# qpc001/Feature_Base_Pointcloud_Registration

Hardware: AMD Instinct MI355X
Metric: registered scans/sec + pose RMSE vs ref, 64×1800 synthetic Velodyne (higher is better)
Workload: dtype f32; 1 GPU; C2: 64x1800 HDL-64-style scans, ~100k-pt local corner+surf map; 1024 independent scan-to-map jobs per GPU per step (C4-style independent jobs); parallelism=single GPU, imu_deskew=False, exact_voxel_order=0

## Files before the change

### feature_base_pointcloud_registration_amd/api.py

```python
import ctypes
import os

import numpy as np

from .fbr_types import (DESKEW_TABLE, IMU_SAMPLE, KEYPOSE, PF_FLOAT32, POINT_XYZI, POINT_XYZIRT, REG_STATS, FbrParams,
                        FbrRegStats, PointCloud2, default_params, ptr)

_HERE = os.path.dirname(os.path.abspath(__file__))
_LIB = None
_VP = ctypes.c_void_p
_I64 = ctypes.c_int64
_I32 = ctypes.c_int32

EXPORTED_SYMBOLS = [
    "fbr_params_default", "fbr_strerror", "fbr_abi_version", "fbr_device_count", "fbr_create",
    "fbr_destroy", "fbr_set_map", "fbr_get_map", "fbr_project", "fbr_extract_features",
    "fbr_register", "fbr_register_trace", "fbr_process_scan", "fbr_reset_stream",
    "fbr_process_batch", "fbr_ingest_bytes", "fbr_debug_counters", "fbr_map_grid_info", "fbr_batch_stage", "fbr_batch_launch", "fbr_batch_wait",
    "fbr_batch_flush", "fbr_batch_export_ready", "fbr_batch_results", "fbr_batch_set_full_masks", "fbr_batch_labels", "fbr_batch_export", "fbr_batch_bytes", "fbr_set_profiling", "fbr_set_profiling_kernels", "fbr_kernel_time", "fbr_stream",
    "fbr_voxel_grid", "fbr_affine_from_pose", "fbr_pose_from_affine", "fbr_selftest_math", "fbr_selftest_eigen6", "fbr_selftest_eig_certified", "fbr_selftest_voxel_order", "fbr_selftest_radix_sort",
    "fbr_load_map", "fbr_pcd_read", "fbr_pcd_write_ascii", "fbr_pcd_write_binary",
    "fbr_msg_to_points", "fbr_points_to_msg_data", "fbr_project_msg", "fbr_process_msg",
    "fbr_imu_convert", "fbr_imu_deskew_info", "fbr_set_deskew", "fbr_stream_copy_bandwidth", "fbr_valu_peak",
    "fbr_keyframe_params_default", "fbr_keyframes_add", "fbr_keyframes_set_pose", "fbr_keyframes_count",
# ... 457 lines not shown
        _check(lib().fbr_ingest_bytes(self._h, ctypes.byref(v)), "fbr_ingest_bytes")
        return v.value

    def batch_stage(self, scans, guesses):
        keep, arr, n_in = self._scan_ptrs(scans)
        g = np.ascontiguousarray(np.asarray(guesses, np.float32).reshape(-1, 6))
        _check(lib().fbr_batch_stage(self._h, arr, ptr(n_in), len(keep), ptr(g)), "fbr_batch_stage")
        self._staged = len(keep)

    def batch_launch(self):
        _check(lib().fbr_batch_launch(self._h), "fbr_batch_launch")

    def batch_wait(self):
        _check(lib().fbr_batch_wait(self._h), "fbr_batch_wait")

    def batch_results(self):
        poses = np.zeros((self._staged, 6), np.float32)
        stats = np.zeros(self._staged, REG_STATS)
        _check(lib().fbr_batch_results(self._h, ptr(poses), ptr(stats)), "fbr_batch_results")
        return poses, stats

    def batch_set_full_masks(self, on=True):
        _check(lib().fbr_batch_set_full_masks(self._h, int(bool(on))), "fbr_batch_set_full_masks")

    def batch_labels(self, job):
        n = _I64()
        rc = lib().fbr_batch_labels(self._h, int(job), None, 0, ctypes.byref(n))
        if rc not in (0, -4):
            _check(rc, "fbr_batch_labels")
        out = np.zeros(max(n.value, 1), np.int8)
        _check(lib().fbr_batch_labels(self._h, int(job), ptr(out), len(out), ctypes.byref(n)), "fbr_batch_labels")
        return out[:n.value]

    def batch_export(self, device_ptr):
        _check(lib().fbr_batch_export(self._h, ctypes.c_void_p(device_ptr)), "fbr_batch_export")

    def batch_flush(self):
        _check(lib().fbr_batch_flush(self._h), "fbr_batch_flush")

    def batch_export_ready(self, device_ptr, wait_stream=0):
        st, lid = _VP(), _I64()
        _check(lib().fbr_batch_export_ready(self._h, ctypes.c_void_p(device_ptr), ctypes.c_void_p(wait_stream or None),
                                            ctypes.byref(st), ctypes.byref(lid)), "fbr_batch_export_ready")
        return lid.value, st.value or 0

    def diag_ring_filter(self, kernel):
        f = lib().fbr_diag_ring_filter
        f.restype, f.argtypes = ctypes.c_int, [_VP, ctypes.c_int]
        _check(f(self._h, int(kernel)), "fbr_diag_ring_filter")

    def diag_force_capacity_error(self, job):
        f = lib().fbr_diag_force_capacity_error
        f.restype, f.argtypes = ctypes.c_int, [_VP, ctypes.c_int]
        _check(f(self._h, int(job)), "fbr_diag_force_capacity_error")

    def batch_bytes(self):
        t, g = ctypes.c_double(), ctypes.c_double()
        _check(lib().fbr_batch_bytes(self._h, ctypes.byref(t), ctypes.byref(g)), "fbr_batch_bytes")
        return t.value, g.value

    def set_profiling(self, on=True, kernels=None):
        names = None if not kernels else ",".join(kernels).encode()
        _check(lib().fbr_set_profiling_kernels(self._h, names), "fbr_set_profiling_kernels")
        _check(lib().fbr_set_profiling(self._h, 1 if on else 0), "fbr_set_profiling")

    def kernel_time(self, name):
# ... 47 lines not shown
```

### feature_base_pointcloud_registration_amd/csrc/fbr_api.hip

```cpp
#include <hip/hip_runtime.h>

#include <algorithm>
#include <atomic>
#include <chrono>
#include <condition_variable>
#include <cmath>
#include <cstdio>
#include <cstdlib>
#include <cstring>
#include <dlfcn.h>
#include <functional>
#include <map>
#include <mutex>
#include <set>
#include <string>
#include <thread>
#include <vector>

#include "fbr_common.h"
#include "fbr_imu.h"
#include "fbr_kernels.h"
#include "fbr_msg.h"

using namespace fbr;
// ... 169 lines not shown
  int8_t* d_fits = nullptr;
  int8_t* d_nsame = nullptr;
  int32_t* d_fb_list = nullptr;
  int32_t* d_bin = nullptr;
  int64_t bin_nb = 0, bin_nb_c = 0;
  unsigned long long* h_iter_flags = nullptr;
  unsigned long long* d_iter_flags = nullptr;
  unsigned long long gn_gen = 0;
  std::set<std::string> profile_only;
  int32_t* d_iter_cnt = nullptr;
  unsigned char* d_feat_scratch = nullptr;
  uint8_t* d_msg = nullptr;
  uint64_t msg_cap = 0;
  bool crop_cached = false;
  bool crop_join = false;
  int32_t* h_crop = nullptr;
  float* h_guess = nullptr;
  int max_items = 0;
  float* d_pose_out = nullptr;
  fbr_reg_stats* d_stats = nullptr;
  float* d_trace = nullptr;
  bool has_map = false;
  DevGrid grid_c, grid_s;
  std::vector<fbr_point_xyzi> map_c_host, map_s_host;
  bool have_projection = false;
  int staged_B = 0;
  std::vector<int64_t> staged_nin;
  double time_last = -1.0;
  bool profiling = false;
  std::map<std::string, KernelTimer> timers;
  std::vector<int32_t> last_iters, last_q, last_n, last_m;
  int items_hint = 0;
  unsigned long long* d_feat_stamps = nullptr;
  fbr_deskew_table* d_desk = nullptr;
  int32_t* d_desk_mode = nullptr;
  int32_t* d_rowmin = nullptr;
  int32_t* d_choff = nullptr;
  DevArena arena;
  bool desk_any = false;
  bool no_time_call = false;
  std::vector<fbr_keypose> kf_poses;
  std::vector<int64_t> kf_c_off, kf_c_cnt, kf_s_off, kf_s_cnt;
  float4 *d_kf_c = nullptr, *d_kf_s = nullptr;
  int64_t kf_c_cap = 0, kf_s_cap = 0, kf_c_used = 0, kf_s_used = 0;
  float4 *d_kraw_c = nullptr, *d_kraw_s = nullptr;
  int64_t kraw_c_cap = 0, kraw_s_cap = 0;
  float4 *d_kds_c = nullptr, *d_kds_s = nullptr;
  int64_t kds_c_n = 0, kds_s_n = 0;
  KfSeg* d_kf_segs = nullptr;
  int64_t kf_segs_cap = 0;
  int* d_bounds = nullptr;
  bool map_nocrop = false;
  int stream_degenerate = 0;
  JobResult* d_result = nullptr;
  JobResult* h_result = nullptr;
  fbr_point_xyzirt* h_scan = nullptr;
  int64_t* h_nin = nullptr;
  uint8_t* h_msg = nullptr;
  uint64_t h_msg_cap = 0;
  Ingest ing;
  JobResult* h_direct = nullptr;
  JobResult* d_direct = nullptr;
  int32_t* d_direct_done = nullptr;
  int32_t direct_gen = 0;
  int32_t direct_gen_seq = 0;
  bool tail_pending = false;
// ... 206 lines not shown
    desk = DeskArgs{c->d_desk_mode + i0, c->d_desk + i0, c->d_rowmin + j0 * c->H};
  const float4* pk = (!sb.stream_mode && !desk.mode && c->staged_pk) ? c->staged_pk + i0 * c->NMAX : nullptr;
  if (!sb.stream_mode && !pk && !c->staged_24) return FBR_ERR_STATE;
  int32_t* owner = c->d_owner + j0 * c->HW;
  OwnerTag ot;
  const int trc = next_owner_tag(c, &ot);
  if (trc) return trc;
  TIMED_ON(c, sb.st, "project", launch_project(sb.st, c->d_pts + i0 * c->NMAX, c->d_nin + i0, c->NMAX, sb.B, c->H,
                                               c->W, owner, c->d_err + j0, sb.stream_mode ? c->single_n : -1, pk, ot));
  TIMED_ON(c, sb.st, "extract",
           launch_extract(sb.st, c->d_pts + i0 * c->NMAX, c->NMAX, owner, sb.B, c->H, c->W, c->d_rowcnt + j0 * c->H,
                          c->d_choff + j0 * c->H * (c->W / 32 + 1),
                          c->d_cloud + j0 * c->HW, c->d_col + j0 * c->HW, c->d_range + j0 * c->HW,
                          c->d_start + j0 * c->H, c->d_end + j0 * c->H, c->d_nvalid + j0, desk, pk, ot));
  return FBR_OK;
}

bool packed_scans_enabled() {
  static const bool v = [] {
    const char* e = std::getenv("FBR_PACKED_SCANS");
    return e ? std::atoi(e) != 0 : true;
  }();
  return v;
}

bool feat_surf_window() {
  static const bool v = [] {
    const char* e = std::getenv("FBR_FEAT_SURF_WINDOW");
    return e ? std::atoi(e) != 0 : true;
  }();
  return v;
}

int stage_features(fbr_ctx* c, const Sub& sb, bool stream_mode, bool err_clear = false, bool labels_out = false) {
  const int64_t j0 = sb.j0, HW = c->HW, H = c->H;
  FeatArgs a{};
  a.B = sb.B;
  a.H = c->H;
  a.W = c->W;
  a.cloud = c->d_cloud + j0 * HW;
  a.col = c->d_col + j0 * HW;
  a.range = c->d_range + j0 * HW;
  a.start_ring = c->d_start + j0 * H;
  a.end_ring = c->d_end + j0 * H;
  a.nvalid = c->d_nvalid + j0;
  a.edge_thr = c->P.edge_threshold;
  a.surf_thr = c->P.surf_threshold;
  if (stream_mode) {
    a.stream = c->d_sstream;
    a.label = c->d_label_stream;
  } else {
    CK(hipMemsetAsync(c->d_sstate + j0, 0, sizeof(StreamState) * sb.B, sb.st));
    a.stream = c->d_sstate + j0;
    a.label = c->d_label + j0 * HW;
  }
  a.corner_slot = c->d_corner_slot + j0 * H * kCornerPerRing;
  a.corner_cnt = c->d_corner_cnt + j0 * H;
  a.err = c->d_err + j0;
  a.surf_full = labels_out || !feat_surf_window() ? 1 : 0;
  a.carry = stream_mode ? 1 : 0;
  a.fresh = stream_mode ? 0 : 1;
  feat_caps(c->W, a);
  a.gscratch = c->d_feat_scratch + j0 * H * a.gslot_bytes;
  a.stamps = c->d_feat_stamps ? c->d_feat_stamps + j0 * H * 12 : nullptr;
  if (!err_clear) CK(hipMemsetAsync(c->d_err + j0, 0, sizeof(int32_t) * sb.B, sb.st));
  TIMED_ON(c, sb.st, "features", launch_features(sb.st, a));
  if (!stream_mode && c->diag_err_job >= sb.in0 && c->diag_err_job < sb.in0 + sb.B)
    CK(hipMemsetD32Async((hipDeviceptr_t)(c->d_err + j0 + (c->diag_err_job - sb.in0)), 1, 1, sb.st));
  VgRing v{};
  v.cloud = a.cloud;
  v.label = a.label;
  v.start_ring = a.start_ring;
  v.end_ring = a.end_ring;
  v.B = sb.B;
  v.H = c->H;
  v.HW = HW;
  v.cap = c->W;
  v.leaf = c->P.odometry_surf_leaf_size;
  v.out = c->d_surf_ring + j0 * HW;
  v.stride_out = c->W;
  v.cnt_out = c->d_surf_ring_cnt + j0 * H;
  v.dbg = std::getenv("FBR_VR_DBG") ? std::atoi(std::getenv("FBR_VR_DBG")) : 0;
  v.exact = c->P.exact_voxel_order ? 1 : 0;
  v.stamps = a.stamps;
  v.kernel = c->diag_ring_filter;
  TIMED_ON(c, sb.st, "voxel_ring", launch_voxel_ring(sb.st, v));
  TIMED_ON(c, sb.st, "concat",
           launch_concat(sb.st, sb.B, c->H, c->W, a.corner_slot, a.corner_cnt, v.out, v.cnt_out,
                         c->d_corner_all + j0 * HW, HW, c->d_ncorner + j0, c->d_surf_all + j0 * HW, HW,
                         c->d_nsurf + j0, c->d_ring_box + j0 * H * kRingBox));
  c->ring_box_valid = true;
  return FBR_OK;
}

GnArgs gn_args(fbr_ctx* c, const Sub& sb, bool trace) {
  const int64_t j0 = sb.j0, HW = c->HW, ib = j0 * c->items_per_job;
  const int mi = std::max(1, c->P.max_iterations);
// ... 911 lines not shown
  if (hipMemset(c->d_sstream, 0, sizeof(StreamState)) != hipSuccess ||
      hipMemset(c->d_label_stream, 0, HW) != hipSuccess || hipMemset(c->d_col, 0, sizeof(int32_t) * Bw * HW) != hipSuccess ||
      hipMemset(c->d_range, 0, sizeof(float) * Bw * HW) != hipSuccess ||
      hipMemset(c->d_desk_mode, 0, sizeof(int32_t) * B) != hipSuccess ||
      hipMemset(c->d_owner, 0x7F, sizeof(int32_t) * Bw * HW) != hipSuccess) {
    fbr_destroy(c);
    return FBR_ERR_HIP;
  }
  c->owner_ib = 1;
  while (((int64_t)1 << c->owner_ib) < c->NMAX) ++c->owner_ib;
  c->owner_tmax = (owner_tags_enabled() && c->owner_ib <= 24) ? ((uint32_t)kEmptyOwner >> c->owner_ib) - 1 : 0;
  if (const char* e = std::getenv("FBR_OWNER_TMAX"))
    if (c->owner_tmax && std::atoi(e) > 0) c->owner_tmax = std::min<uint32_t>(c->owner_tmax, (uint32_t)std::atoi(e));
  *out = c;
  return FBR_OK;
}

int fbr_destroy(fbr_ctx* c) {
  if (!c) return FBR_ERR_INVALID_ARG;
  (void)hipSetDevice(c->dev);
  if (c->stream) (void)fbr_sync(c->stream);
  for (int k = 1; k < kMaxSub; ++k)
    if (c->xstream[k]) (void)fbr_sync(c->xstream[k]);
  void* ptrs[] = {c->d_pts, c->d_nin, c->d_guess, c->d_owner, c->d_rowcnt, c->d_col, c->d_start, c->d_end,
                  c->d_nvalid, c->d_cloud, c->d_range, c->d_sstate, c->d_sstream, c->d_label, c->d_label_stream,
                  c->d_corner_slot, c->d_corner_cnt, c->d_surf_ring, c->d_surf_ring_cnt, c->d_ring_box,
                  c->d_err, c->d_corner_all, c->d_surf_all, c->d_cornerDS, c->d_surfDS, c->d_ncorner, c->d_nsurf,
                  c->d_ncds, c->d_nsds, c->d_vg_scratch, c->d_gn, c->d_items, c->d_nitems,
                  c->d_item_range, c->d_cropcnt, c->d_cropwork, c->d_partial, c->d_pose_out, c->d_stats, c->d_trace, c->d_nbr, c->d_fitc, c->d_fits, c->d_nsame, c->d_fb_list, c->d_bin, c->d_iter_cnt, c->d_feat_scratch, c->d_msg,
                  c->d_desk, c->d_desk_mode, c->d_rowmin, c->d_choff,
                  c->d_kf_c, c->d_kf_s, c->d_kraw_c, c->d_kraw_s, c->d_kds_c, c->d_kds_s, c->d_kf_segs, c->d_bounds, c->d_direct_done, c->d_pk};
  for (void* p : ptrs)
    if (p) (void)hipFree(p);
  if (c->h_iter_flags) (void)hipHostFree(c->h_iter_flags);
  free_grid(c->grid_c);
  free_grid(c->grid_s);
  arena_free(c->arena);
  for (void* h : {(void*)c->h_result, (void*)c->h_scan, (void*)c->h_nin, (void*)c->h_msg, (void*)c->h_crop, (void*)c->h_guess,
                  (void*)c->h_direct})
    if (h) (void)hipHostFree(h);
  if (c->d_result) (void)hipFree(c->d_result);
  if (c->ing.cstream) (void)fbr_sync(c->ing.cstream);
  if (c->ing.xstream) (void)fbr_sync(c->ing.xstream);
  if (c->ing.h_stage) (void)hipHostFree(c->ing.h_stage);
  if (c->ing.d_pts_slot[1]) (void)hipFree(c->ing.d_pts_slot[1]);
  for (uint8_t* d : c->ing.d_stage)
    if (d) (void)hipFree(d);
  if (c->ing.copied_ev) (void)hipEventDestroy(c->ing.copied_ev);
  if (c->ing.d_nin) (void)hipFree(c->ing.d_nin);
  if (c->ing.h_nin) (void)hipHostFree(c->ing.h_nin);
  for (auto& e : c->ing.up_ev)
    if (e) (void)hipEventDestroy(e);
  for (auto& e : c->ing.chunk_ev)
    if (e) (void)hipEventDestroy(e);
  if (c->ing.cstream) (void)hipStreamDestroy(c->ing.cstream);
  if (c->ing.xstream) (void)hipStreamDestroy(c->ing.xstream);
  for (auto& kv : c->timers) {
    for (auto& pr : kv.second.pending) {
      (void)hipEventDestroy(pr.first);
      (void)hipEventDestroy(pr.second);
    }
    for (auto& pr : kv.second.pool) {
      (void)hipEventDestroy(pr.first);
      (void)hipEventDestroy(pr.second);
    }
  }
// ... 984 lines not shown
  return FBR_OK;
}

int fbr_ingest_bytes(fbr_ctx* c, double* h2d_bytes) {
  if (!c || !h2d_bytes) return FBR_ERR_INVALID_ARG;
  *h2d_bytes = c->ing.h2d_bytes;
  return FBR_OK;
}

int fbr_voxel_grid(fbr_ctx* c, const fbr_point_xyzi* in, int64_t n, float leaf, fbr_point_xyzi* out, int64_t* n_out) {
  if (!c || n < 0 || (n && !in) || !(leaf > 0)) return FBR_ERR_INVALID_ARG;
  CK(enter(c));
  std::vector<fbr_point_xyzi> o;
  int rc = voxel_grid_once(c, in, n, leaf, o);
  if (rc) return rc;
  if (out) std::memcpy(out, o.data(), sizeof(fbr_point_xyzi) * o.size());
  if (n_out) *n_out = (int64_t)o.size();
  return FBR_OK;
}

extern "C" int fbr_diag_feature_stamps(fbr_ctx* c, unsigned long long* out ) {
  if (!c) return FBR_ERR_INVALID_ARG;
  CK(enter(c));
  const size_t n = (size_t)c->Bwork * c->H * 12;
  if (!c->d_feat_stamps) {
    CK(hipMalloc(&c->d_feat_stamps, sizeof(unsigned long long) * n));
    CK(hipMemset(c->d_feat_stamps, 0, sizeof(unsigned long long) * n));
    return FBR_OK;
  }
  if (out) CK(fbr_memcpy_sync(out, c->d_feat_stamps, sizeof(unsigned long long) * n, hipMemcpyDeviceToHost));
  return FBR_OK;
}

int fbr_set_profiling(fbr_ctx* c, int enable) {
  if (!c) return FBR_ERR_INVALID_ARG;
  c->profiling = enable != 0;
  return FBR_OK;
}

int fbr_set_profiling_kernels(fbr_ctx* c, const char* names) {
  if (!c) return FBR_ERR_INVALID_ARG;
  c->profile_only.clear();
  if (!names) return FBR_OK;
  std::string cur;
  for (const char* q = names;; ++q) {
    if (*q == ',' || *q == '\0') {
      if (!cur.empty()) c->profile_only.insert(cur);
      cur.clear();
      if (*q == '\0') break;
    } else {
      cur.push_back(*q);
    }
  }
  return FBR_OK;
}

int fbr_kernel_time(fbr_ctx* c, const char* kernel, double* total_ms, int64_t* launches) {
  if (!c || !kernel) return FBR_ERR_INVALID_ARG;
  CK(enter(c));
  auto itr = c->timers.find(kernel);
  if (itr == c->timers.end()) {
    if (total_ms) *total_ms = 0.0;
    if (launches) *launches = 0;
    return FBR_OK;
  }
  KernelTimer& t = itr->second;
// ... 213 lines not shown
```

### feature_base_pointcloud_registration_amd/csrc/fbr_kernels.h

```cpp
#pragma once
#include <hip/hip_ext.h>
#include <hip/hip_runtime.h>
#include <stdint.h>

#include <algorithm>
#include <atomic>

#include "fbr_common.h"

namespace fbr {

struct LaunchTimer {
  hipEvent_t start = nullptr, stop = nullptr;
  int launched = 0;
};
inline LaunchTimer& launch_timer() {
  static thread_local LaunchTimer t;
  return t;
}

struct DebugCounters {
  std::atomic<long long> launches{0}, host_syncs{0}, flag_polls{0};
  std::atomic<long long> host_ns[4] = {0, 0, 0, 0};
  std::atomic<long long> batch_ns[2] = {0, 0};
// ... 38 lines not shown
struct DeskArgs {
  const int32_t* mode;
  const fbr_deskew_table* table;
  int32_t* rowmin;
};
void launch_extract(hipStream_t s, const fbr_point_xyzirt* pts, int64_t nmax, int32_t* owner, int B, int H,
                    int W, int32_t* rowcnt, int32_t* choff, float4* cloud, int32_t* col, float* range,
                    int32_t* start_ring, int32_t* end_ring, int32_t* nvalid, const DeskArgs& desk,
                    const float4* pk, const OwnerTag& ot);

struct FeatArgs {
  int B, H, W;
  const float4* cloud;
  const int32_t* col;
  const float* range;
  const int32_t* start_ring;
  const int32_t* end_ring;
  const int32_t* nvalid;
  float edge_thr, surf_thr;
  StreamState* stream;
  int8_t* label;
  float4* corner_slot;
  int32_t* corner_cnt;
  int32_t* err;
  int lcap, segcap;
  int kseg;
  int nwcap;
  unsigned char* gscratch;
  int64_t gslot_bytes;
  unsigned long long* stamps;
  int surf_full = 1;
  int carry = 0;
  int fresh = 0;
};
size_t features_lds_bytes(const FeatArgs& a, int nwv);
size_t features_gslot_bytes(const FeatArgs& a);
void launch_features(hipStream_t s, const FeatArgs& a);

struct VgSet {
  const float4* in;
  int64_t stride_in;
  const int32_t* cnt_in;
  int64_t cap;
  float4* out;
  int64_t stride_out;
  int32_t* cnt_out;
  uint32_t* scratch;
  float leaf;
  int nseg;
  int morton;
  int exact;
  const float* box;
  int box_n;
  int64_t box_stride;
};
constexpr int64_t kVgScratch = 5;
struct VgArgs {
  VgSet s[2];
  int32_t* err = nullptr;
};
constexpr int32_t kVgErrLookback = 16;
constexpr int64_t kVgLdsCap = 4096;
void launch_voxel_grid(hipStream_t s, const VgArgs& a);

struct DevArena {
  char* base = nullptr;
// ... 166 lines not shown
```

### feature_base_pointcloud_registration_amd/csrc/k_features.hip

```cpp
#include "fbr_common.h"
#include "fbr_kernels.h"
#include "fbr_sort.h"

#include <algorithm>
#include <cstdlib>
#include <type_traits>

namespace fbr {

__device__ __forceinline__ void wsync() {
  __builtin_amdgcn_fence(__ATOMIC_SEQ_CST, "workgroup");
  __builtin_amdgcn_wave_barrier();
}

namespace {
constexpr uint64_t kPadKey = kF64KeyMax;
constexpr int kSurfWindow = 64;
constexpr int kWin = 256 + 16;
constexpr int kWinBytes = kWin * (sizeof(float) + sizeof(int16_t));
}

struct Bits {
  uint64_t* w;
  __device__ __forceinline__ bool get(int i) const { return (w[i >> 6] >> (i & 63)) & 1ull; }
// ... 111 lines not shown
                              const FeatArgs& a, int job, const uint64_t* frz = nullptr) {
  const int nwm = (m >> 6) + 1;
  uint32_t cmr[WMAX];
#pragma unroll
  for (int w = 0; w < WMAX; ++w) cmr[w] = (w < nwm && 64 * w + lane <= m) ? cmbits(64 * w + lane) : 0u;
  for (int round = 0;; ++round) {
    bool any = false, progress = false;
#pragma unroll
    for (int w = 0; w < WMAX; ++w) {
      const uint64_t live = frz ? und[w] & ~frz[w] : und[w];
      if (w < nwm && live != 0ull) {
        bool nt = false, tk = false;
        const bool mine = (live >> lane) & 1ull;
        if (mine) {
          const uint32_t wt = win10(w > 0 ? tak[w - 1] : 0ull, tak[w], w + 1 < WMAX ? tak[w + 1] : 0ull, lane);
          const uint32_t wu = win10(w > 0 ? und[w - 1] : 0ull, und[w], w + 1 < WMAX ? und[w + 1] : 0ull, lane);
          if (wt & cmr[w]) nt = true;
          else if (!(wu & cmr[w])) tk = true;
        }
        const uint64_t bt = __ballot(tk);
        tak[w] |= bt;
        if (bt != 0ull && mine && !tk && !nt) {
          const uint32_t wt = win10(w > 0 ? tak[w - 1] : 0ull, tak[w], w + 1 < WMAX ? tak[w + 1] : 0ull, lane);
          nt = (wt & cmr[w]) != 0u;
        }
        const uint64_t bn = __ballot(nt);
        und[w] &= ~(bt | bn);
        progress |= (bt | bn) != 0ull;
        any |= (frz ? und[w] & ~frz[w] : und[w]) != 0ull;
      }
    }
    if (!any || (frz && !progress)) break;
    if (round > 4 * (m + 2)) {
      if (lane == 0) atomicOr(&a.err[job], 8);
      break;
    }
  }
}

__device__ __forceinline__ int wave_partition(SmoothEntry* a, int lo, int hi, float p, uint16_t* posL, uint16_t* posR,
                                              int lane) {
  int cntL = 0;
  for (int b = lo; b < hi; b += 64) {
    const int i = b + lane;
    const bool isL = i < hi && !(a[i].v < p);
    const uint64_t bl = __ballot(isL);
    if (isL) posL[cntL + __popcll(bl & ((1ull << lane) - 1ull))] = (uint16_t)i;
    cntL += __popcll(bl);
  }
  int cntR = 0;
  for (int t = hi - 1; t >= lo; t -= 64) {
    const int i = t - lane;
    const bool isR = i >= lo && !(p < a[i].v);
    const uint64_t br = __ballot(isR);
    if (isR) posR[cntR + __popcll(br & ((1ull << lane) - 1ull))] = (uint16_t)i;
    cntR += __popcll(br);
  }
  wsync();
  const int mn = min(cntL, cntR);
  int K1 = 0;
  for (int k0 = 0; k0 < mn; k0 += 64) {
    const int k = k0 + lane;
    const uint64_t bo = __ballot(k < mn && posL[k] < posR[k]);
    K1 += __popcll(bo);
    if (bo != ~0ull) break;
  }
// ... 352 lines not shown
    uint64_t mk = S.occc.w[c] | A;
#pragma unroll
    for (int d = 1; d <= 5; ++d) mk |= (A >> d) | (An << (64 - d));
#pragma unroll
    for (int d = 1; d <= 6; ++d) mk |= (B << d) | (Bp >> (64 - d));
    if (c == 0 && S.wlo == 0)
      for (int k = 0; k < 5 && k < S.L; ++k)
        if (st->picked04[k]) mk |= 1ull << k;
    S.picked.w[c] = mk;
  }
  __syncthreads();
  FBR_STAMP(1);

  int corner_cnt = 0;
  float4* corner_out = a.corner_slot + (int64_t)slot * kCornerPerRing;
  constexpr int kCq = WMAX;
  float cpf[kCq];
  int pf_seg = -1, pf_next = -1, pf_len = 0;
  auto prefetch_curv = [&](int j0) __attribute__((always_inline)) {
    pf_next = -1;
    for (int jj = j0; jj < 6; ++jj) {
      const int psp = (s * (6 - jj) + e * jj) / 6, pep = (s * (5 - jj) + e * (jj + 1)) / 6 - 1;
      if (psp >= pep) continue;
      const int pb = max(psp - S.wlo - 6, 0), pl = min(pep - S.wlo + 7, S.L) - pb;
      if (pl > 64 * kCq || pep - psp + 1 > segcap) return;
#pragma unroll
      for (int q = 0; q < kCq; ++q) cpf[q] = S.gcurv[pb + min(64 * q + lane, pl - 1)];
      pf_next = jj;
      pf_len = pl;
      return;
    }
  };
  int lastj = -1;
  for (int j = 0; j < 6; j++)
    if ((s * (6 - j) + e * j) / 6 < (s * (5 - j) + e * (j + 1)) / 6 - 1) lastj = j;
  for (int j = 0; j < 6; j++) {
    const int sp = (s * (6 - j) + e * j) / 6;
    const int ep = (s * (5 - j) + e * (j + 1)) / 6 - 1;
    if (sp >= ep) continue;
    const int m = ep - sp;
    if (m + 1 > segcap || m > kseg) {
      if (tid == 0) atomicOr(&a.err[job], 2);
      return;
    }
    S.sbase = max(sp - S.wlo - 6, 0);
    const int slen = min(ep - S.wlo + 7, S.L) - S.sbase;
    if (pf_seg != j)
      for (int t = tid; t < slen; t += NT) S.scurv[t] = S.gcurv[S.sbase + t];
    __syncthreads();
#ifdef FBR_FEAT_SKIP_STALE
    const bool has_stale = false;
#else
    const bool has_stale = (sp <= 4 && 4 < ep);
#endif
    auto sorted_order = [&]() __attribute__((always_inline)) {
      int kpow = 1;
      while (kpow < m) kpow <<= 1;
      for (int t = lane; t < kpow; t += 64) {
        uint64_t key = kPadKey;
        if (t < m) {
          const int pos = sp + t;
          const float v = (pos == 4) ? st->smooth4_value : S.scurv[pos - S.wlo - S.sbase];
          key = ((uint64_t)__float_as_uint(v) << 16) | (uint64_t)t;
        }
        S.keys[t] = key;
      }
      wsync();
      bitonic_sort_keys<QP>(S.keys, kpow, lane);
      bool tflag = false, nflag = false;
      for (int t = lane; t < m; t += 64) {
        const uint32_t vb = (uint32_t)(S.keys[t] >> 16);
        nflag |= vb > 0x7f800000u;
        if (t + 1 < m) tflag |= (uint32_t)(S.keys[t + 1] >> 16) == vb;
      }
      const bool nan = __any(nflag);
      const bool tie = __any(tflag) || nan;
      FBR_STAMP(2);
      if (tie) {
        SmoothEntry* A = nan ? S.seg : (SmoothEntry*)S.rb;
        for (int t = lane; t < m; t += 64) {
          const int pos = sp + t;
          A[t] = (pos == 4) ? SmoothEntry{st->smooth4_value, st->smooth4_ind} : SmoothEntry{S.scurv[pos - S.wlo - S.sbase], pos};
        }
        wsync();
        if (nan) {
          if (lane == 0) std_sort_emul(S.seg, m, S.sstack);
          wsync();
        } else {
// ... 49 lines not shown
        }
        wsync();
      }
    };
    float* tlv = (float*)S.rb;
    uint16_t* tlu = (uint16_t*)(tlv + segcap);
    uint16_t* vis = tlu + segcap;
    auto cm_member = [&](int u) __attribute__((always_inline)) -> bool {
      const int li = sp - S.wlo + u;
      const int f = reach_fwd(S, li), b = reach_bwd(S, li);
      float cv[11];
#pragma unroll
      for (int d = 0; d < 11; ++d) cv[d] = S.scurv[max(li + d - 5, 0) - S.sbase];
      const float vu = cv[5];
      const int lf = min(f, m - u), lb = min(b, u);
      const uint32_t nbf = ((1u << lf) - 1u) << 5, nbb = ((1u << lb) - 1u) << (5 - lb);
      const uint32_t epb = (m - u >= 1 && m - u <= 5) ? 1u << (4 + m - u) : 0u;
      uint32_t gt = 0, eq = 0;
#pragma unroll
      for (int d = 1; d <= 5; ++d) {
        gt |= (cv[5 + d] > vu ? 1u : 0u) << (4 + d);
        eq |= (!(cv[5 + d] < vu || cv[5 + d] > vu) ? 1u : 0u) << (4 + d);
        gt |= (cv[5 - d] > vu ? 1u : 0u) << (5 - d);
        eq |= (!(cv[5 - d] < vu || cv[5 - d] > vu) ? 1u : 0u) << (5 - d);
      }
      const uint32_t notep = u != m ? ~0u : 0u;
      const uint32_t nb = nbf | nbb;
      const uint32_t hc = ((gt | epb) & nbf) | (gt & nbb & notep);
      S.cm[u] = hc | (nb << 10) | ((uint32_t)f << 20) | ((uint32_t)b << 24);
      return ((eq & ~epb & nbf) | (eq & nbb & notep)) != 0u;
    };
    const bool seg_full = a.surf_full || (a.carry && sp <= 9);
    const bool cm_sparse = !seg_full && !has_stale;
    bool direct = !has_stale;
#ifdef FBR_FEAT_SKIP_CM
    if (direct) {
      for (int u = tid; u <= m; u += NT) S.cm[u] = 0u;
      __syncthreads();
    }
    if (false) {
#else
    if (direct) {
#endif
      bool tf = false;
      int nlist = m + 1;
      if (cm_sparse) {
        uint16_t* list = (uint16_t*)S.rb;
        if (wv == 0) {
          int cnt = 0;
          const int wlo_u = j == lastj ? m + 1 : max(0, m - (kSurfWindow - 1));
          for (int k0 = 0; k0 <= m; k0 += 64) {
            const int u = k0 + lane;
            bool need = false;
            if (u <= m) {
              const int li = sp + u - S.wlo;
              need = u >= wlo_u || (!S.picked.get(li) && S.edgec.get(li));
            }
            const uint64_t bm = __ballot(need);
            if (need) list[cnt + __popcll(bm & ((1ull << lane) - 1ull))] = (uint16_t)u;
            cnt += __popcll(bm);
          }
          if (lane == 0) S.tmask[15] = (uint64_t)cnt;
        }
        if constexpr (NWV == 1) wsync();
        else __syncthreads();
        nlist = (int)S.tmask[15];
      }
      for (int k0 = 64 * wv; k0 < nlist; k0 += NT) {
        if (cm_sparse) {
          const int k = k0 + lane;
          if (k < nlist) tf |= cm_member(((const uint16_t*)S.rb)[k]);
        } else {
          const int u = k0 + lane;
          if (u <= m) tf |= cm_member(u);
        }
      }
      if constexpr (NWV == 1) {
        direct = !__any(tf);
        wsync();
      } else {
        __syncthreads();
        direct = !__syncthreads_or(tf);
      }
      FBR_STAMP(10);
    }
    if (wv == 0) {
    if (!direct) sorted_order();
    FBR_STAMP(3);
    if (has_stale) {
      SmoothEntry* ent = (SmoothEntry*)S.rb;
      for (int k = lane; k <= m; k += 64) ent[k] = S.seg[k];
      wsync();
      if (!stale_walks_fast(S, slen, ent, a, m, CL, corner_out, corner_cnt, S.cm,
                               (int32_t*)(ent + segcap), lane)) {
        if (lane == 0) serial_walks(S, slen, ent, a, job, m, CL, corner_out, corner_cnt);
        corner_cnt = __shfl(corner_cnt, 0);
        wsync();
      }
    } else {
      uint64_t und[WMAX], tak[WMAX];
      auto corner_walk = [&]() __attribute__((always_inline)) {
#pragma unroll
        for (int w = 0; w < WMAX; ++w) {
          const int u = 64 * w + lane;
          bool cand = false;
          if (u <= m) {
            const int li = sp + u - S.wlo;
            cand = !S.picked.get(li) && S.edgec.get(li);
          }
          und[w] = __ballot(cand);
          tak[w] = 0ull;
        }
#ifndef FBR_FEAT_SKIP_CORNER
        greedy_rounds(m, lane, und, tak, [&](int u) { return S.cm[u] & 1023u; }, a, job);
#endif
      };
      corner_walk();
      FBR_STAMP(4);
      int T = 0;
      if (direct) {
#pragma unroll
        for (int w = 0; w < WMAX; ++w) {
          if ((tak[w] >> lane) & 1ull) {
            const int q = T + __popcll(tak[w] & ((1ull << lane) - 1ull));
            const int u = 64 * w + lane;
            tlu[q] = (uint16_t)u;
            tlv[q] = S.scurv[sp + u - S.wlo - S.sbase];
          }
          T += __popcll(tak[w]);
        }
        wsync();
        bool tf = false;
        for (int c = lane; c < T; c += 64) {
          const int u = tlu[c];
          const float vu = tlv[c];
          int rank = 0;
          for (int c2 = 0; c2 < T; ++c2) {
            const int u2 = tlu[c2];
            const float v2 = tlv[c2];
            if (u2 == m) rank += (u != m);
            else if (u != m && c2 != c) {
              if (v2 > vu) ++rank;
              else if (!(v2 < vu)) tf = true;
            }
          }
          vis[rank] = (uint16_t)u;
        }
        if (__any(tf)) {
          direct = false;
          wsync();
          sorted_order();
          corner_walk();
        }
        wsync();
        FBR_STAMP(11);
      }
      if (lane < WMAX) {
        uint64_t t = 0;
#pragma unroll
        for (int w = 0; w < WMAX; ++w)
          if (w == lane) t = tak[w];
        S.tmask[lane] = t;
      }
      wsync();
      const int R = direct ? T : m + 1;
      int taken = 0;
      for (int r0 = 0; r0 < R && taken < kCornerPerSeg; r0 += 64) {
        const int rr = r0 + lane;
        int u = -1;
        if (rr < R) u = direct ? (int)vis[rr] : (int)S.sorder[rr == 0 ? m : m - rr];
        const bool acc = u >= 0 && ((S.tmask[u >> 6] >> (u & 63)) & 1ull);
        const uint64_t mk = __ballot(acc);
        const int pos = taken + __popcll(mk & ((1ull << lane) - 1ull));
        if (acc && pos < kCornerPerSeg) {
          corner_out[corner_cnt + pos] = CL[sp + u];
          const int li = sp + u - S.wlo;
          const uint32_t c = S.cm[u];
          atomicOr((unsigned long long*)&S.labpos.w[li >> 6], 1ull << (li & 63));
          or_range(S.picked, li - (int)((c >> 24) & 15u), li + (int)((c >> 20) & 15u));
        }
        taken += __popcll(mk);
      }
      corner_cnt += min(taken, kCornerPerSeg);
      wsync();
      FBR_STAMP(5);
      if constexpr (NWV == 1) prefetch_curv(j + 1);
      const bool bnd = !seg_full;
      const int ulo = bnd ? max(0, m - (kSurfWindow - 1)) : 0;
      auto surf_cand = [&](bool window) __attribute__((always_inline)) {
#pragma unroll
        for (int w = 0; w < WMAX; ++w) {
          const int u = 64 * w + lane;
          bool cand = false;
          if (u <= m && (!window || u >= ulo - 5)) {
            const int li = sp + u - S.wlo;
            cand = !S.picked.get(li) && S.surfc.get(li);
          }
          und[w] = __ballot(cand);
          tak[w] = 0ull;
        }
      };
      auto surf_cm = [&](int u) {
        const uint32_t c = S.cm[u];
        return ((c >> 10) & 1023u) & ~(c & 1023u);
      };
      if (bnd && j == lastj) {
#pragma unroll
        for (int w = 0; w < WMAX; ++w) tak[w] = 0ull;
      } else {
        surf_cand(bnd && ulo > 0);
#ifndef FBR_FEAT_SKIP_SURF
        if (bnd && ulo > 0) {
          uint64_t frz[WMAX];
#pragma unroll
          for (int w = 0; w < WMAX; ++w) {
            const int u = 64 * w + lane;
            frz[w] = und[w] & __ballot(u < ulo);
          }
          greedy_rounds(m, lane, und, tak, surf_cm, a, job, frz);
          bool open = false;
#pragma unroll
          for (int w = 0; w < WMAX; ++w) {
            const int u = 64 * w + lane;
            open |= u >= m - 4 && u <= m && ((und[w] >> lane) & 1ull) && !((frz[w] >> lane) & 1ull);
          }
          if (__any(open)) {
            if (direct) {
              bool tf2 = false;
              for (int u = lane; u <= m; u += 64) tf2 |= cm_member(u);
              wsync();
              if (__any(tf2)) sorted_order();
            }
            surf_cand(false);
            greedy_rounds(m, lane, und, tak, surf_cm, a, job);
          }
        } else {
          greedy_rounds(m, lane, und, tak, surf_cm, a, job);
        }
#endif
      }
      FBR_STAMP(6);
#pragma unroll
      for (int w = 0; w < WMAX; ++w) {
        const int u = 64 * w + lane;
        if (u <= m && ((tak[w] >> lane) & 1ull)) {
          const int li = sp + u - S.wlo;
          const uint32_t c = S.cm[u];
          atomicOr((unsigned long long*)&S.labneg.w[li >> 6], 1ull << (li & 63));
          or_range(S.picked, li - (int)((c >> 24) & 15u), li + (int)((c >> 20) & 15u));
        }
      }
      pf_seg = pf_next;
      if (pf_seg >= 0) {
#pragma unroll
        for (int q = 0; q < kCq; ++q)
          if (64 * q + lane < pf_len) S.scurv[64 * q + lane] = cpf[q];
      }
      wsync();
    }
    FBR_STAMP(7);
    FBR_STAMP(8);
    }
    if constexpr (NWV > 1) __syncthreads();
  }
  if constexpr (NWV > 1) __syncthreads();
  int8_t* LB = a.label + job * HW;
  for (int k = max(cb, 0) + tid; k < ca; k += NT) {
    const int li = k - S.wlo;
    const int8_t lab = S.labpos.get(li) ? 1 : (S.labneg.get(li) ? -1 : 0);
    if (k >= 5 && k < n - 5) LB[k] = lab;
    else if (k < 5 && (lab != 0 || a.fresh)) LB[k] = lab;
  }
  if (cb <= 0 && tid < 5 && tid < S.L) st->picked04[tid] = S.picked.get(tid) ? 1 : 0;
  if (tid == 0) a.corner_cnt[slot] = corner_cnt;
#ifdef FBR_FEAT_STAMPS
  FBR_STAMP(9);
  if (tid == 0 && a.stamps)
    for (int i = 0; i < 12; ++i) a.stamps[(int64_t)slot * 12 + i] = stamp_acc[i];
#endif
}

size_t features_lds_bytes(const FeatArgs& a, int nwv) {
  const size_t region_b = std::max<size_t>((size_t)nwv * kWinBytes, (size_t)8 * a.segcap + sizeof(int32_t) * kCornerPerSeg);
  return (size_t)((a.segcap + 19) & ~3) * sizeof(float) + (size_t)9 * a.nwcap * sizeof(uint64_t) + sizeof(uint64_t) * 16 +
         sizeof(SortFrame) * kSortStack + sizeof(uint32_t) * a.segcap + 16 + region_b;
}

size_t features_gslot_bytes(const FeatArgs& a) {
  const size_t b = sizeof(uint64_t) * a.kseg + 2 * sizeof(SmoothEntry) * a.segcap + 2 * sizeof(uint16_t) * a.segcap +
                   16 + sizeof(float) * a.lcap;
  return (b + 255) & ~(size_t)255;
}

int feature_waves(int rings) {
  static const int forced = [] {
    const char* e = std::getenv("FBR_FEAT_WAVES");
    const int v = e ? std::atoi(e) : 0;
    return v >= 4 ? 4 : v >= 2 ? 2 : v == 1 ? 1 : 0;
  }();
  if (forced) return forced;
  return rings <= 2048 ? 4 : 1;
}

void launch_features(hipStream_t s, const FeatArgs& a) {
  const int nwv = feature_waves(a.B * a.H);
  const dim3 grid(a.B * a.H);
  if (nwv == 1 && a.segcap <= 5 * 64 && a.kseg <= 4 * 128) {
// ... 18 lines not shown
```

Baseline: 142,700 scans/s.

## Add compacted-candidate greedy selection for corner and surface feature picking

Adds a compact path in the feature kernel. Corner candidates are gathered into a dense list of at most 128, and the greedy non-maximum suppression rounds run over one or two 64-bit masks using precomputed 11-bit neighbour conflict masks, instead of sweeping WMAX words over the whole segment. Surface selection in the bounded window gets the same treatment and falls back to the generic path when the window is still open. The surface window default becomes 59 and the path is switched by env vars. Also adds a diagnostic path-record buffer and API, which is off unless allocated.

```diff
diff --git a/feature_base_pointcloud_registration_amd/api.py b/feature_base_pointcloud_registration_amd/api.py
--- a/feature_base_pointcloud_registration_amd/api.py
+++ b/feature_base_pointcloud_registration_amd/api.py
@@ -513,6 +513,15 @@
         _check(lib().fbr_batch_labels(self._h, int(job), ptr(out), len(out), ctypes.byref(n)), "fbr_batch_labels")
         return out[:n.value]
 
+    def feature_paths(self):
+        f = lib().fbr_diag_feature_paths
+        f.restype, f.argtypes = ctypes.c_int, [_VP, _VP, _I64, _VP]
+        n = _I64()
+        _check(f(self._h, None, 0, ctypes.byref(n)), "fbr_diag_feature_paths")
+        out = np.zeros(max(n.value, 1), np.uint32)
+        _check(f(self._h, ptr(out), len(out), ctypes.byref(n)), "fbr_diag_feature_paths")
+        return out[:n.value].reshape(-1, self.params.n_scan)
+
     def batch_export(self, device_ptr):
         _check(lib().fbr_batch_export(self._h, ctypes.c_void_p(device_ptr)), "fbr_batch_export")
 
diff --git a/feature_base_pointcloud_registration_amd/csrc/fbr_api.hip b/feature_base_pointcloud_registration_amd/csrc/fbr_api.hip
--- a/feature_base_pointcloud_registration_amd/csrc/fbr_api.hip
+++ b/feature_base_pointcloud_registration_amd/csrc/fbr_api.hip
@@ -225,6 +225,7 @@
   std::vector<int32_t> last_iters, last_q, last_n, last_m;
   int items_hint = 0;
   unsigned long long* d_feat_stamps = nullptr;
+  uint32_t* d_feat_paths = nullptr;
   fbr_deskew_table* d_desk = nullptr;
   int32_t* d_desk_mode = nullptr;
   int32_t* d_rowmin = nullptr;
@@ -497,6 +498,24 @@
   return v;
 }
 
+bool feat_compact() {
+  static const bool v = [] {
+    const char* e = std::getenv("FBR_FEAT_COMPACT");
+    return e ? std::atoi(e) != 0 : true;
+  }();
+  return v;
+}
+
+constexpr int kFeatSurfWinDefault = 59;
+int feat_surf_win() {
+  static const int v = [] {
+    const char* e = std::getenv("FBR_FEAT_SURF_WIN");
+    const int w = e ? std::atoi(e) : kFeatSurfWinDefault;
+    return w == 59 ? 59 : 64;
+  }();
+  return v;
+}
+
 int stage_features(fbr_ctx* c, const Sub& sb, bool stream_mode, bool err_clear = false, bool labels_out = false) {
   const int64_t j0 = sb.j0, HW = c->HW, H = c->H;
   FeatArgs a{};
@@ -528,6 +547,9 @@
   feat_caps(c->W, a);
   a.gscratch = c->d_feat_scratch + j0 * H * a.gslot_bytes;
   a.stamps = c->d_feat_stamps ? c->d_feat_stamps + j0 * H * 12 : nullptr;
+  a.compact = feat_compact() ? 1 : 0;
+  a.surf_win = feat_surf_win();
+  a.paths = c->d_feat_paths ? c->d_feat_paths + j0 * H : nullptr;
   if (!err_clear) CK(hipMemsetAsync(c->d_err + j0, 0, sizeof(int32_t) * sb.B, sb.st));
   TIMED_ON(c, sb.st, "features", launch_features(sb.st, a));
   if (!stream_mode && c->diag_err_job >= sb.in0 && c->diag_err_job < sb.in0 + sb.B)
@@ -1505,6 +1527,7 @@
                   c->d_kf_c, c->d_kf_s, c->d_kraw_c, c->d_kraw_s, c->d_kds_c, c->d_kds_s, c->d_kf_segs, c->d_bounds, c->d_direct_done, c->d_pk};
   for (void* p : ptrs)
     if (p) (void)hipFree(p);
+  if (c->d_feat_paths) (void)hipFree(c->d_feat_paths);
   if (c->h_iter_flags) (void)hipHostFree(c->h_iter_flags);
   free_grid(c->grid_c);
   free_grid(c->grid_s);
@@ -2555,6 +2578,24 @@
   return FBR_OK;
 }
 
+extern "C" int fbr_diag_feature_paths(fbr_ctx* c, uint32_t* out, int64_t cap, int64_t* n_out) {
+  if (!c) return FBR_ERR_INVALID_ARG;
+  CK(enter(c));
+  const size_t n = (size_t)c->Bwork * c->H;
+  if (n_out) *n_out = (int64_t)n;
+  if (!c->d_feat_paths) {
+    CK(hipMalloc(&c->d_feat_paths, sizeof(uint32_t) * n));
+    CK(hipMemset(c->d_feat_paths, 0, sizeof(uint32_t) * n));
+    return FBR_OK;
+  }
+  if (!out) return FBR_OK;
+  if (cap < (int64_t)n) return FBR_ERR_CAPACITY;
+  CK(hipDeviceSynchronize());
+  CK(fbr_memcpy_sync(out, c->d_feat_paths, sizeof(uint32_t) * n, hipMemcpyDeviceToHost));
+  CK(hipMemset(c->d_feat_paths, 0, sizeof(uint32_t) * n));
+  return FBR_OK;
+}
+
 int fbr_set_profiling(fbr_ctx* c, int enable) {
   if (!c) return FBR_ERR_INVALID_ARG;
   c->profiling = enable != 0;
diff --git a/feature_base_pointcloud_registration_amd/csrc/fbr_kernels.h b/feature_base_pointcloud_registration_amd/csrc/fbr_kernels.h
--- a/feature_base_pointcloud_registration_amd/csrc/fbr_kernels.h
+++ b/feature_base_pointcloud_registration_amd/csrc/fbr_kernels.h
@@ -94,6 +94,9 @@
   int surf_full = 1;
   int carry = 0;
   int fresh = 0;
+  int compact = 1;
+  int surf_win = 59;
+  uint32_t* paths = nullptr;
 };
 size_t features_lds_bytes(const FeatArgs& a, int nwv);
 size_t features_gslot_bytes(const FeatArgs& a);
diff --git a/feature_base_pointcloud_registration_amd/csrc/k_features.hip b/feature_base_pointcloud_registration_amd/csrc/k_features.hip
--- a/feature_base_pointcloud_registration_amd/csrc/k_features.hip
+++ b/feature_base_pointcloud_registration_amd/csrc/k_features.hip
@@ -167,6 +167,69 @@
     }
     if (!any || (frz && !progress)) break;
     if (round > 4 * (m + 2)) {
+      if (lane == 0) atomicOr(&a.err[job], 8);
+      break;
+    }
+  }
+}
+
+struct U128 {
+  uint64_t lo, hi;
+};
+
+__device__ __forceinline__ U128 place11(uint32_t rel, int pos) {
+  const int s = pos - 5;
+  U128 r;
+  if (s < 0) {
+    r.lo = (uint64_t)(rel >> (-s));
+    r.hi = 0ull;
+  } else if (s < 64) {
+    r.lo = (uint64_t)rel << s;
+    r.hi = s > 53 ? (uint64_t)rel >> (64 - s) : 0ull;
+  } else {
+    r.lo = 0ull;
+    r.hi = (uint64_t)rel << (s - 64);
+  }
+  return r;
+}
+
+__device__ __forceinline__ uint64_t readlane64(uint64_t v, int l);
+
+__device__ __forceinline__ uint64_t member_bits(uint64_t wv, int sh, int k, int m) {
+  const uint64_t lo = readlane64(wv, k), hi = readlane64(wv, k + 1);
+  const uint64_t x = sh ? (lo >> sh) | (hi << (64 - sh)) : lo;
+  const int rem = m - 64 * k;
+  return rem >= 63 ? x : (rem < 0 ? 0ull : x & ((2ull << rem) - 1ull));
+}
+
+template <int NH>
+__device__ __forceinline__ void compact_rounds(int lane, uint64_t& und0, uint64_t& und1, uint64_t& tak0, uint64_t& tak1,
+                                               const U128 (&cf)[NH], uint64_t frz0, int cap, const FeatArgs& a, int job) {
+  for (int round = 0;; ++round) {
+    bool progress = false;
+#pragma unroll
+    for (int h = 0; h < NH; ++h) {
+      const uint64_t live = h == 0 ? und0 & ~frz0 : und1;
+      if (live != 0ull) {
+        const bool mine = (live >> lane) & 1ull;
+        const uint64_t clo = cf[h].lo, chi = NH > 1 ? cf[h].hi : 0ull;
+        bool nt = false, tk = false;
+        if (mine) {
+          if (((tak0 & clo) | (tak1 & chi)) != 0ull) nt = true;
+          else if (((und0 & clo) | (und1 & chi)) == 0ull) tk = true;
+        }
+        const uint64_t bt = __ballot(tk);
+        if (h == 0) tak0 |= bt;
+        else tak1 |= bt;
+        if (bt != 0ull && mine && !tk && !nt) nt = ((tak0 & clo) | (tak1 & chi)) != 0ull;
+        const uint64_t bn = __ballot(nt);
+        if (h == 0) und0 &= ~(bt | bn);
+        else und1 &= ~(bt | bn);
+        progress |= (bt | bn) != 0ull;
+      }
+    }
+    if (((und0 & ~frz0) | und1) == 0ull || !progress) break;
+    if (round > cap) {
       if (lane == 0) atomicOr(&a.err[job], 8);
       break;
     }
@@ -585,6 +648,7 @@
     }
   };
   int lastj = -1;
+  uint32_t rec = 0u;
   for (int j = 0; j < 6; j++)
     if ((s * (6 - j) + e * j) / 6 < (s * (5 - j) + e * (j + 1)) / 6 - 1) lastj = j;
   for (int j = 0; j < 6; j++) {
@@ -606,7 +670,15 @@
 #else
     const bool has_stale = (sp <= 4 && 4 < ep);
 #endif
+    uint16_t* cl = (uint16_t*)(S.rb + 4 * segcap);
+    int nc_pre = -1;
+    const int li0 = sp - S.wlo;
+    auto cand_words = [&]() __attribute__((always_inline)) {
+      const int w = (li0 >> 6) + lane;
+      return (lane <= WMAX && w < S.nw) ? ~S.picked.w[w] & S.edgec.w[w] : 0ull;
+    };
     auto sorted_order = [&]() __attribute__((always_inline)) {
+      nc_pre = -1;
       int kpow = 1;
       while (kpow < m) kpow <<= 1;
       for (int t = lane; t < kpow; t += 64) {
@@ -722,6 +794,7 @@
     };
     const bool seg_full = a.surf_full || (a.carry && sp <= 9);
     const bool cm_sparse = !seg_full && !has_stale;
+    const int swin = a.compact ? a.surf_win : kSurfWindow;
     bool direct = !has_stale;
 #ifdef FBR_FEAT_SKIP_CM
     if (direct) {
@@ -737,19 +810,23 @@
       if (cm_sparse) {
         uint16_t* list = (uint16_t*)S.rb;
         if (wv == 0) {
-          int cnt = 0;
-          const int wlo_u = j == lastj ? m + 1 : max(0, m - (kSurfWindow - 1));
-          for (int k0 = 0; k0 <= m; k0 += 64) {
-            const int u = k0 + lane;
-            bool need = false;
-            if (u <= m) {
-              const int li = sp + u - S.wlo;
-              need = u >= wlo_u || (!S.picked.get(li) && S.edgec.get(li));
-            }
-            const uint64_t bm = __ballot(need);
-            if (need) list[cnt + __popcll(bm & ((1ull << lane) - 1ull))] = (uint16_t)u;
-            cnt += __popcll(bm);
-          }
+          int cnt = 0, ncand = 0;
+          const int wlo_u = j == lastj ? m + 1 : max(0, m - (swin - 1));
+          const uint64_t cwv = cand_words();
+          const uint64_t ltm0 = (1ull << lane) - 1ull;
+          for (int k = 0; 64 * k <= m; ++k) {
+            const uint64_t cb = member_bits(cwv, li0 & 63, k, m);
+            const int lo = wlo_u - 64 * k;
+            const int rem = m - 64 * k;
+            uint64_t wb = lo <= 0 ? ~0ull : (lo >= 64 ? 0ull : ~0ull << lo);
+            if (rem < 63) wb &= (2ull << rem) - 1ull;
+            const uint64_t nb = cb | wb;
+            if ((nb >> lane) & 1ull) list[cnt + __popcll(nb & ltm0)] = (uint16_t)(64 * k + lane);
+            if ((cb >> lane) & 1ull) cl[ncand + __popcll(cb & ltm0)] = (uint16_t)(64 * k + lane);
+            cnt += __popcll(nb);
+            ncand += __popcll(cb);
+          }
+          nc_pre = ncand;
           if (lane == 0) S.tmask[15] = (uint64_t)cnt;
         }
         if constexpr (NWV == 1) wsync();
@@ -775,6 +852,7 @@
       FBR_STAMP(10);
     }
     if (wv == 0) {
+    rec |= 1u << (24 + j);
     if (!direct) sorted_order();
     FBR_STAMP(3);
     if (has_stale) {
@@ -787,9 +865,88 @@
         corner_cnt = __shfl(corner_cnt, 0);
         wsync();
       }
+      rec |= 15u << (4 * j);
     } else {
-      uint64_t und[WMAX], tak[WMAX];
-      auto corner_walk = [&]() __attribute__((always_inline)) {
+      int T = 0;
+      int ccode = 0;
+      const uint64_t ltm = (1ull << lane) - 1ull;
+      auto corner_compact = [&]() __attribute__((always_inline)) -> bool {
+        int nc = nc_pre;
+        if (nc < 0) {
+          nc = 0;
+          const uint64_t cwv = cand_words();
+          for (int k = 0; 64 * k <= m; ++k) {
+            const uint64_t cb = member_bits(cwv, li0 & 63, k, m);
+            if ((cb >> lane) & 1ull) cl[nc + __popcll(cb & ltm)] = (uint16_t)(64 * k + lane);
+            nc += __popcll(cb);
+          }
+        }
+        if (nc > 128) return false;
+        T = 0;
+        ccode = nc > 64 ? 1 : 0;
+        if (nc == 0 && direct) return true;
+        wsync();
+        auto run = [&](auto NHc) __attribute__((always_inline)) {
+          constexpr int NH = decltype(NHc)::value;
+          U128 cf[NH];
+          int uu[NH];
+#pragma unroll
+          for (int h = 0; h < NH; ++h) {
+            const int q = 64 * h + lane;
+            uint32_t rel = 0u;
+            int u = 0;
+            if (q < nc) {
+              u = cl[q];
+              const uint32_t c10 = S.cm[u] & 1023u;
+              int un[10];
+#pragma unroll
+              for (int k = 1; k <= 5; ++k) {
+                un[4 + k] = cl[min(q + k, nc - 1)];
+                un[5 - k] = cl[max(q - k, 0)];
+              }
+#pragma unroll
+              for (int k = 1; k <= 5; ++k) {
+                const int df = min(un[4 + k] - u, 6), db = min(u - un[5 - k], 6);
+                if (q + k < nc && df <= 5 && ((c10 >> (4 + df)) & 1u)) rel |= 1u << (5 + k);
+                if (q - k >= 0 && db <= 5 && ((c10 >> (5 - min(db, 5))) & 1u)) rel |= 1u << (5 - k);
+              }
+            }
+            uu[h] = u;
+            cf[h] = place11(rel, q);
+          }
+          uint64_t und0 = nc >= 64 ? ~0ull : (1ull << nc) - 1ull;
+          uint64_t und1 = NH > 1 ? (nc >= 128 ? ~0ull : (1ull << (nc - 64)) - 1ull) : 0ull;
+          uint64_t tak0 = 0ull, tak1 = 0ull;
+#ifndef FBR_FEAT_SKIP_CORNER
+          compact_rounds<NH>(lane, und0, und1, tak0, tak1, cf, 0ull, 4 * (nc + 2), a, job);
+#endif
+          T = __popcll(tak0) + __popcll(tak1);
+          if (!direct) {
+            if (lane < WMAX) S.tmask[lane] = 0ull;
+            wsync();
+          }
+#pragma unroll
+          for (int h = 0; h < NH; ++h) {
+            const uint64_t th = h == 0 ? tak0 : tak1;
+            if ((th >> lane) & 1ull) {
+              const int u = uu[h];
+              if (direct) {
+                const int q = (h == 0 ? 0 : __popcll(tak0)) + __popcll(th & ltm);
+                tlu[q] = (uint16_t)u;
+                tlv[q] = S.scurv[sp + u - S.wlo - S.sbase];
+              } else {
+                atomicOr((unsigned long long*)&S.tmask[u >> 6], 1ull << (u & 63));
+              }
+            }
+          }
+          wsync();
+        };
+        if (nc <= 64) run(std::integral_constant<int, 1>{});
+        else run(std::integral_constant<int, 2>{});
+        return true;
+      };
+      auto corner_generic = [&]() __attribute__((always_inline)) {
+        uint64_t und[WMAX], tak[WMAX];
 #pragma unroll
         for (int w = 0; w < WMAX; ++w) {
           const int u = 64 * w + lane;
@@ -804,22 +961,35 @@
 #ifndef FBR_FEAT_SKIP_CORNER
         greedy_rounds(m, lane, und, tak, [&](int u) { return S.cm[u] & 1023u; }, a, job);
 #endif
+        T = 0;
+        ccode = 2;
+        if (direct) {
+#pragma unroll
+          for (int w = 0; w < WMAX; ++w) {
+            if ((tak[w] >> lane) & 1ull) {
+              const int q = T + __popcll(tak[w] & ltm);
+              const int u = 64 * w + lane;
+              tlu[q] = (uint16_t)u;
+              tlv[q] = S.scurv[sp + u - S.wlo - S.sbase];
+            }
+            T += __popcll(tak[w]);
+          }
+        }
+        if (lane < WMAX) {
+          uint64_t t = 0;
+#pragma unroll
+          for (int w = 0; w < WMAX; ++w)
+            if (w == lane) t = tak[w];
+          S.tmask[lane] = t;
+        }
+        wsync();
+      };
+      auto corner_walk = [&]() __attribute__((always_inline)) {
+        if (!(a.compact && corner_compact())) corner_generic();
       };
       corner_walk();
       FBR_STAMP(4);
-      int T = 0;
       if (direct) {
-#pragma unroll
-        for (int w = 0; w < WMAX; ++w) {
-          if ((tak[w] >> lane) & 1ull) {
-            const int q = T + __popcll(tak[w] & ((1ull << lane) - 1ull));
-            const int u = 64 * w + lane;
-            tlu[q] = (uint16_t)u;
-            tlv[q] = S.scurv[sp + u - S.wlo - S.sbase];
-          }
-          T += __popcll(tak[w]);
-        }
-        wsync();
         bool tf = false;
         for (int c = lane; c < T; c += 64) {
           const int u = tlu[c];
@@ -845,21 +1015,13 @@
         wsync();
         FBR_STAMP(11);
       }
-      if (lane < WMAX) {
-        uint64_t t = 0;
-#pragma unroll
-        for (int w = 0; w < WMAX; ++w)
-          if (w == lane) t = tak[w];
-        S.tmask[lane] = t;
-      }
-      wsync();
       const int R = direct ? T : m + 1;
       int taken = 0;
       for (int r0 = 0; r0 < R && taken < kCornerPerSeg; r0 += 64) {
         const int rr = r0 + lane;
         int u = -1;
         if (rr < R) u = direct ? (int)vis[rr] : (int)S.sorder[rr == 0 ? m : m - rr];
-        const bool acc = u >= 0 && ((S.tmask[u >> 6] >> (u & 63)) & 1ull);
+        const bool acc = u >= 0 && (direct || ((S.tmask[u >> 6] >> (u & 63)) & 1ull));
         const uint64_t mk = __ballot(acc);
         const int pos = taken + __popcll(mk & ((1ull << lane) - 1ull));
         if (acc && pos < kCornerPerSeg) {
@@ -876,31 +1038,37 @@
       FBR_STAMP(5);
       if constexpr (NWV == 1) prefetch_curv(j + 1);
       const bool bnd = !seg_full;
-      const int ulo = bnd ? max(0, m - (kSurfWindow - 1)) : 0;
-      auto surf_cand = [&](bool window) __attribute__((always_inline)) {
-#pragma unroll
-        for (int w = 0; w < WMAX; ++w) {
-          const int u = 64 * w + lane;
-          bool cand = false;
-          if (u <= m && (!window || u >= ulo - 5)) {
-            const int li = sp + u - S.wlo;
-            cand = !S.picked.get(li) && S.surfc.get(li);
-          }
-          und[w] = __ballot(cand);
-          tak[w] = 0ull;
-        }
-      };
+      const int ulo = bnd ? max(0, m - (swin - 1)) : 0;
       auto surf_cm = [&](int u) {
         const uint32_t c = S.cm[u];
         return ((c >> 10) & 1023u) & ~(c & 1023u);
       };
-      if (bnd && j == lastj) {
-#pragma unroll
-        for (int w = 0; w < WMAX; ++w) tak[w] = 0ull;
-      } else {
-        surf_cand(bnd && ulo > 0);
+      auto surf_apply = [&](int u) __attribute__((always_inline)) {
+        const int li = sp + u - S.wlo;
+        const uint32_t c = S.cm[u];
+        atomicOr((unsigned long long*)&S.labneg.w[li >> 6], 1ull << (li & 63));
+        or_range(S.picked, li - (int)((c >> 24) & 15u), li + (int)((c >> 20) & 15u));
+      };
+      auto surf_generic = [&](bool window, bool rest) __attribute__((always_inline)) -> int {
+        uint64_t und[WMAX], tak[WMAX];
+        auto surf_cand = [&](bool win) __attribute__((always_inline)) {
+#pragma unroll
+          for (int w = 0; w < WMAX; ++w) {
+            const int u = 64 * w + lane;
+            bool cand = false;
+            if (u <= m && (!win || u >= ulo - 5)) {
+              const int li = sp + u - S.wlo;
+              cand = !S.picked.get(li) && S.surfc.get(li);
+            }
+            und[w] = __ballot(cand);
+            tak[w] = 0ull;
+          }
+        };
+        int code = rest ? 2 : 3;
+        bool whole = true;
 #ifndef FBR_FEAT_SKIP_SURF
-        if (bnd && ulo > 0) {
+        if (window) {
+          surf_cand(true);
           uint64_t frz[WMAX];
 #pragma unroll
           for (int w = 0; w < WMAX; ++w) {
@@ -914,32 +1082,75 @@
             const int u = 64 * w + lane;
             open |= u >= m - 4 && u <= m && ((und[w] >> lane) & 1ull) && !((frz[w] >> lane) & 1ull);
           }
-          if (__any(open)) {
-            if (direct) {
-              bool tf2 = false;
-              for (int u = lane; u <= m; u += 64) tf2 |= cm_member(u);
-              wsync();
-              if (__any(tf2)) sorted_order();
-            }
-            surf_cand(false);
-            greedy_rounds(m, lane, und, tak, surf_cm, a, job);
-          }
+          whole = __any(open);
+          code = whole ? 2 : 1;
+          rest = whole;
+        }
+        if (whole) {
+          if (rest && direct) {
+            bool tf2 = false;
+            for (int u = lane; u <= m; u += 64) tf2 |= cm_member(u);
+            wsync();
+            if (__any(tf2)) sorted_order();
+          }
+          surf_cand(false);
+          greedy_rounds(m, lane, und, tak, surf_cm, a, job);
+        }
+#else
+        surf_cand(false);
+#endif
+        FBR_STAMP(6);
+#pragma unroll
+        for (int w = 0; w < WMAX; ++w) {
+          const int u = 64 * w + lane;
+          if (u <= m && ((tak[w] >> lane) & 1ull)) surf_apply(u);
+        }
+        return code;
+      };
+      auto surf_compact = [&]() __attribute__((always_inline)) -> bool {
+        const int base = max(0, ulo - 5);
+        const bool two = m - base >= 64;
+        const int u0 = base + lane, u1 = base + 64 + lane;
+        const int lb = li0 + base, wb = (lb >> 6) + lane;
+        const uint64_t swv = (lane < 3 && wb < S.nw) ? ~S.picked.w[wb] & S.surfc.w[wb] : 0ull;
+        uint64_t und0 = member_bits(swv, lb & 63, 0, m - base);
+        uint64_t und1 = two ? member_bits(swv, lb & 63, 1, m - base) : 0ull;
+        const uint64_t frz0 = und0 & ((1ull << (ulo - base)) - 1ull);
+        uint64_t tak0 = 0ull, tak1 = 0ull;
+        auto rel_of = [&](int u) __attribute__((always_inline)) {
+          const uint32_t s10 = surf_cm(u);
+          return (s10 & 31u) | ((s10 >> 5) << 6);
+        };
+#ifndef FBR_FEAT_SKIP_SURF
+        const bool live0 = ((und0 & ~frz0) >> lane) & 1ull;
+        if (!two) {
+          U128 cf[1];
+          cf[0] = place11(live0 ? rel_of(u0) : 0u, lane);
+          compact_rounds<1>(lane, und0, und1, tak0, tak1, cf, frz0, 4 * (m - base + 2), a, job);
         } else {
-          greedy_rounds(m, lane, und, tak, surf_cm, a, job);
-        }
+          U128 cf[2];
+          cf[0] = place11(live0 ? rel_of(u0) : 0u, lane);
+          cf[1] = place11(((und1 >> lane) & 1ull) ? rel_of(u1) : 0u, 64 + lane);
+          compact_rounds<2>(lane, und0, und1, tak0, tak1, cf, frz0, 4 * (m - base + 2), a, job);
+        }
+        const bool open = (u0 >= m - 4 && u0 <= m && (((und0 & ~frz0) >> lane) & 1ull)) ||
+                          (u1 >= m - 4 && u1 <= m && ((und1 >> lane) & 1ull));
+        if (__any(open)) return false;
 #endif
-      }
-      FBR_STAMP(6);
-#pragma unroll
-      for (int w = 0; w < WMAX; ++w) {
-        const int u = 64 * w + lane;
-        if (u <= m && ((tak[w] >> lane) & 1ull)) {
-          const int li = sp + u - S.wlo;
-          const uint32_t c = S.cm[u];
-          atomicOr((unsigned long long*)&S.labneg.w[li >> 6], 1ull << (li & 63));
-          or_range(S.picked, li - (int)((c >> 24) & 15u), li + (int)((c >> 20) & 15u));
-        }
-      }
+        FBR_STAMP(6);
+        if ((tak0 >> lane) & 1ull) surf_apply(u0);
+        if ((tak1 >> lane) & 1ull) surf_apply(u1);
+        return true;
+      };
+      int scode = 0;
+      if (bnd && j == lastj) {
+        FBR_STAMP(6);
+      } else if (bnd && a.compact) {
+        scode = surf_compact() ? 1 : surf_generic(false, ulo > 0);
+      } else {
+        scode = surf_generic(bnd && ulo > 0, false);
+      }
+      rec |= (uint32_t)(ccode | (scode << 2)) << (4 * j);
       pf_seg = pf_next;
       if (pf_seg >= 0) {
 #pragma unroll
@@ -963,6 +1174,7 @@
   }
   if (cb <= 0 && tid < 5 && tid < S.L) st->picked04[tid] = S.picked.get(tid) ? 1 : 0;
   if (tid == 0) a.corner_cnt[slot] = corner_cnt;
+  if (tid == 0 && a.paths) a.paths[slot] = rec;
 #ifdef FBR_FEAT_STAMPS
   FBR_STAMP(9);
   if (tid == 0 && a.stamps)
```

Measured after the change: 146,900 scans/s (median of 6 runs). 1.03x the previous value.
